# YukeWang96/GNNAdvisor_OSDI21

Hardware: AMD Instinct MI355X
Metric: aggregated edges/sec, GCN sum-aggregation SpMM (SAG) hidden=64 (higher is better)
Workload: dtype f32; 1 GPU; reddit-like power-law graph, random node order; num_nodes=232965, nnz=114623790, dim=64, partSize=128, num_parts=1008217, parallelism=single GPU, call=GNNA.SAG (pybind module, reference signature, fresh output), decider=auto/mi355x, column_phases=16, build_id=0.6.1+70ede4b55f79bb39

## Files before the change

### gnnadvisor_osdi21_amd/csrc/gnna_agg.hip

```cpp
#include <hip/hip_runtime.h>

#include <algorithm>
#include <cmath>
#include <cstdint>
#include <cstdio>

#include "gnna.h"
#include "gnna_device.h"
#include "gnna_internal.h"

namespace gnna {
namespace {


__global__ void __launch_bounds__(kBlock)
prologue_kernel(float *__restrict__ Y, size_t n_floats, int D, int ldy, const int32_t *__restrict__ p2n,
                const int32_t *__restrict__ pp, int64_t P, int32_t *flag, int32_t seq, int validate, int zero_fill,
                const int32_t *__restrict__ chk_ids, int64_t chk_n, const unsigned long long *__restrict__ chk_sum,
                int32_t *stale_flag, uint32_t *__restrict__ clear_words, int n_clear)
{
    if (blockIdx.x == 0 && (int)threadIdx.x < n_clear) clear_words[threadIdx.x] = 0u;
    const unsigned fill_blocks = chk_ids ? gridDim.x - 1 : gridDim.x;
    if (blockIdx.x >= fill_blocks) {
        if (threadIdx.x < kWave) {
// ... 261 lines not shown
    if (st.edges <= 0 || half_rows < 256.0) return 0.0;
    const double pos = std::min(23.0, 2.0 * std::log2(half_rows / 256.0));
    const int k = (int)pos;
    const double lo = st.near[k], hi = st.near[std::min(23, k + 1)];
    return (lo + (hi - lo) * (pos - k)) / st.edges;
}

int sweep_auto_phases(const gnna_tuning &t, int mode, int dim, size_t x_bytes, int64_t num_out_rows, int64_t num_in_rows,
                      const SlicePlanStats &st, int B, int num_cus, bool deterministic, int part_size)
{
    const double edges = st.edges;
    if (t.sweep != 0 || deterministic || B < 2) return 0;
    if (dim <= 32 || dim > 64 || !sweep_supports(mode, dim, x_bytes)) return 0;
    if (num_in_rows != num_out_rows || x_bytes > ((size_t)160 << 20)) return 0;
    if (edges < 300.0 * (double)std::max<int64_t>(1, num_out_rows)) return 0;
    const double cap = (double)sweep_acc_rows(dim, 1) * 0.9 * (double)std::max(8, num_cus);
    if ((double)num_out_rows > 2.0 * cap) return 0;
    if (near_share(st, (double)num_in_rows / 16.0) > 0.30) return 0;
    if (t.column_phases >= 2) return B;
    return std::max(2, std::min(std::min(16, 2 * B), std::max(2, part_size / 4)));
}

constexpr double kDenseEdgeSeconds = 9.9e-12;
constexpr double kDenseChunkSeconds = 0.97e-6;
constexpr double kDenseLaunchSeconds = 7.0e-6;
constexpr double kDenseMinSaving = 25.0e-6;
constexpr double kDenseMinShare = 0.03;

int trimmed_hubs(int H, int num_cus)
{
    const int round = kDenseTileRanks * std::max(1, num_cus);
    return (H > round && H % round != 0 && H % round < round / 4) ? H / round * round : H;
}

double dense_block_saving(double hubs, double entries, int num_cus)
{
    if (hubs <= 0.0) return 0.0;
    const double He = (double)trimmed_hubs((int)hubs, num_cus);
    const double Hp = std::ceil(He / kDenseChunkRanks) * kDenseChunkRanks;
    const double rounds = std::ceil(Hp / kDenseTileRanks / (double)std::max(1, num_cus));
    const double kept = entries * (He / hubs) * (He / hubs);
    return kept * kDenseEdgeSeconds - rounds * (Hp / kDenseChunkRanks) * kDenseChunkSeconds - kDenseLaunchSeconds;
}

bool dense_block_pays(double saving, double entries, double edges) { return saving > kDenseMinSaving && entries >= kDenseMinShare * edges; }

int sweep_phases_of_width(const gnna_tuning &t, int dim, size_t foot_bytes, size_t x_bytes, int64_t num_out_rows,
                          int64_t num_in_rows, const SlicePlanStats &st, int B, int num_cus, int partSize, int S)
{
    int Bs = sweep_auto_phases(t, MODE_SAG, dim, foot_bytes, num_out_rows, num_in_rows, st, B, num_cus, t.deterministic == 1, partSize);
    if (t.sweep == 1 && t.deterministic != 1 && sweep_supports(MODE_SAG, dim, x_bytes))
        Bs = t.column_phases >= 2 ? B : std::max(2, std::min(std::min(16, 2 * B), std::max(2, partSize / 4)));
    return std::min(Bs, S);
}

int choose_slices(const SlicePlanStats &st, size_t x_bytes, int S, uint32_t slice_rows, int64_t num_out_rows,
                  bool square, bool hinted_scattered)
{
    if (st.groups <= 0 || st.edges <= 0) return 1;
    if (!hinted_scattered) {
        if (square) {
            const double row_bytes = (double)x_bytes / ((double)slice_rows * S);
            const double half_rows = 1.75 * 1048576.0 / row_bytes;
            const bool long_rows_cached = st.edges >= 200.0 * (double)std::max<int64_t>(1, num_out_rows) && x_bytes <= (size_t)250000000;
            const bool one_line_rows = row_bytes > 64.0 && row_bytes <= 128.0;
// ... 304 lines not shown
            rc = get_packed_ids(ds, stream, db.res_plan, Bs, kWave, false, false, &res_ids, &res_off);
            if (rc != GNNA_OK) return rc;
            dense = true;
        }
        uint32_t *sync = ds->sweep_sync + (size_t)call_block_of(ds, stream, seq) * kSweepSlotWords;
        static_assert(kXcds * 16 + 2 <= kBlock, "the prologue clears the sweep counters with one block");
        rc = run_prologue(0, sync, kXcds * 16 + 2);
        if (rc != GNNA_OK) return rc;
        SweepLaunch w;
        w.mode = mode; w.X = X; w.col = column_index; w.pp = part_pointers; w.p2n = part2Node; w.Y = out;
        w.cnt = cnt; w.row_scale = row_scale; w.flag = flag; w.seq = seq; w.trust = tune.trust_canonical ? 1 : 0; w.sync = sync;
        w.P = num_parts; w.D = dim; w.ldx = ldx; w.ldy = ldy; w.S = S; w.B = Bs;
        w.relu = relu; w.num_out_rows = num_nodes;
        w.U = std::max(tune.loads_in_flight, 8);
        w.rows_with_edges = plan.stats.valid ? (int64_t)std::min((double)num_nodes, plan.stats.groups) : num_nodes;
        if (tune.groups_per_chunk > 64) w.rounds = tune.groups_per_chunk / 64;
        w.slack = tune.sweep_slack; w.wgs_per_cu = tune.blocks_per_cu;
        w.dynamic = tune.xcd_remap != 0;
        w.plain_ok = !accumulate_into_out; w.eps = eps;
        w.ids_packed = sw_ids; w.item_off = sw_off; w.packed_stale = stale_flag;
        if (dense) { w.res_col = db.res_col; w.res_pp = db.res_pp; w.res_cnt = db.res_cnt; w.res_ids_packed = res_ids; w.res_item_off = res_off; }
        t_last_phases = Bs;
        t_last_launches = 1;
        rc = launch_sweep(ds, w, stream);
        if (rc != GNNA_OK) return rc;
        if (dense) {
            rc = launch_hub_block(ds, stream, db, X, ldx, out, ldy, dim, mode == MODE_GIN, eps, row_scale, stale_flag, seq);
            if (rc != GNNA_OK) return rc;
        }
        profile_record(prof_call, 2, stream);
        return GNNA_OK;
    }

    int G = std::min(64, tune.groups_per_chunk * B);
    if (mode == MODE_EDGE && cnt && !windowed && plan.handle && plan.pinned && (plan.stats.valid || tune.sweep == 1) &&
        tune.xcd_remap != 0) {
        const int Bs = sweep_phases_of_width(tune, dim, foot_bytes, x_bytes, num_nodes, num_in_rows, plan.stats, B, ds->num_cus,
                                             partSize, S);
        if (Bs >= 2) { B = Bs; G = kWave; }
    }
    t_last_phases = B;
    StreamLaunch a;
    a.mode = mode; a.X = X; a.col = column_index; a.pp = part_pointers; a.p2n = part2Node; a.Y = out;
    a.cnt = cnt; a.row_scale = row_scale; a.flag = flag; a.seq = seq;
    if (mode == MODE_EDGE) { a.deg_row = nullptr; a.deg_col = nullptr; a.edge_w = degrees_in; }
    else { a.deg_row = degrees; a.deg_col = degrees_in; }
    a.trust = tune.trust_canonical ? 1 : 0; a.P = num_parts;
    a.D = dim; a.ldx = ldx; a.ldy = ldy; a.G = G; a.U = tune.loads_in_flight; a.S = S; a.B = B;
    a.win_lo = win_lo; a.win_hi = win_hi; a.relu = relu; a.num_out_rows = num_nodes;
    t_last_launches = 1;
// ... 206 lines not shown
    if (num_parts < 0 || num_in_rows < 0 || num_out_rows < 0 || partSize <= 0 || num_dims < 0 || (num_dims > 0 && !dims))
        return fail(GNNA_ERR_INVALID_ARGUMENT, "gnna_prepare_graph: bad argument");
    for (int i = 0; i < num_dims; i++)
        if (phases_out) phases_out[i] = 1;
    if (num_parts == 0) return GNNA_OK;
    if (!column_index || !part_pointers || !part2Node) return fail(GNNA_ERR_INVALID_ARGUMENT, "null index pointer");
    hipStream_t stream = static_cast<hipStream_t>(stream_v);
    hipStreamCaptureStatus cap = hipStreamCaptureStatusNone;
    (void)hipStreamIsCapturing(stream, &cap);
    if (cap != hipStreamCaptureStatusNone)
        return fail(GNNA_ERR_UNSUPPORTED, "gnna_prepare_graph synchronises and allocates: call it before the capture");
    DeviceState *ds = nullptr;
    int rc = get_device_state(&ds);
    if (rc != GNNA_OK) return rc;
    drain_dead_buffers();
    LaunchGuard in_flight;
    SlicePlan plan;
    rc = get_slice_plan(ds, stream, column_index, part_pointers, part2Node, num_parts, num_in_rows, true, true, &plan);
    if (rc != GNNA_OK) return rc;
    if (!plan.cnt || !plan.stats.valid) return fail(GNNA_ERR_HIP, "gnna_prepare_graph: the slice plan could not be built");
    gnna_tuning tune;
    gnna_get_tuning(&tune);
    const bool hot = plan.stats.edges >= 32.0 * (double)num_in_rows;
    size_t staged = 0, det_bytes = 0;
    std::vector<std::pair<int, int>> widths;
    for (int i = 0; i < num_dims; i++) {
        if (dims[i] <= 0) return fail(GNNA_ERR_INVALID_ARGUMENT, "gnna_prepare_graph: dims[%d] = %d", i, dims[i]);
        const int nb = column_blocks(tune, dims[i], num_in_rows, (int64_t)plan.stats.edges);
        if (nb <= 1) { widths.emplace_back(i, dims[i]); continue; }
        const int w = ((dims[i] + nb - 1) / nb + 3) / 4 * 4;
        widths.emplace_back(i, w);
        if (dims[i] % w) widths.emplace_back(i, dims[i] % w);
    }
    for (const auto &wd : widths) {
        const int i = wd.first;
        const int dim = wd.second;
        gnna_tuning t = tune;
        apply_graph_hints(column_index, dims[i], &t);
        const size_t raw = (size_t)num_in_rows * (size_t)dim * sizeof(float);
        const bool hot_rows = hot && raw <= ((size_t)1 << 30);
        const int ldx = pick_row_stride(t, dim, hot_rows, num_in_rows, true);
        const size_t x_bytes = (size_t)num_in_rows * (size_t)ldx * sizeof(float);
        const size_t foot_bytes = gather_footprint_bytes(num_in_rows, ldx, dim);
        if (hot_rows || t.gcn_prescale == 1 || ldx != dim) staged = std::max(staged, x_bytes);
        int B = 1;
        const bool can_slice = num_parts >= 1024 && num_in_rows >= 64 && foot_bytes >= ((size_t)2 << 20);
        {
            if (t.column_phases >= 2 && num_in_rows >= kMaxSlices) B = std::min(t.column_phases, kMaxSlices);
            else if (t.column_phases == 0 && can_slice && foot_bytes >= ((size_t)6 << 20))
                B = choose_slices(plan.stats, foot_bytes, plan.S, plan.slice_rows, num_out_rows, num_in_rows == num_out_rows,
                                  t.nonlocal_ids == 1);
        }
        const bool first_of_width = &wd == &widths.front() || (&wd - 1)->first != i;
        if (phases_out) phases_out[i] = first_of_width ? std::max(1, B) : std::max(phases_out[i], std::max(1, B));
        if (B >= 2 && t.pack_ids != 2 && plan.handle) {
            const int32_t *ids = nullptr; const uint32_t *off = nullptr;
            const int Bs = sweep_phases_of_width(t, dim, foot_bytes, x_bytes, num_out_rows, num_in_rows, plan.stats, B, ds->num_cus,
                                                 partSize, plan.S);
            const bool swept = Bs >= 2 && t.xcd_remap != 0;
            if (swept) rc = get_packed_ids(ds, stream, plan.handle, Bs, kWave, true, true, &ids, &off);
            if (rc == GNNA_OK && (!swept || t.gcn_prescale == 2))
                rc = get_packed_ids(ds, stream, plan.handle, B, std::max(1, std::min(kWave, t.groups_per_chunk * B)), true, true, &ids, &off);
            if (rc != GNNA_OK) return rc;
            if (phases_out && Bs >= 2) phases_out[i] = first_of_width ? Bs : std::max(phases_out[i], Bs);
            const int dense_mode = dense_block_mode();
            const bool self_swept = t.sweep == 0 && t.column_phases < 2;
            {
                DenseBlock have;
                if (plan_dense_block(plan.handle, &have) && have.off != (dense_mode == 0)) {
                    have.off = dense_mode == 0;
                    plan_set_dense_block(plan.handle, have);
                }
            }
            if (swept && ids && dense_mode != 0 && dim >= kDenseMinDim && dim <= kDenseMaxDim && num_in_rows == num_out_rows &&
                (dense_mode == 2 || self_swept)) {
                DenseBlock db;
                if (!plan_dense_block(plan.handle, &db) && db.declined_mode != dense_mode) {
                    rc = build_dense_block(ds, stream, column_index, part_pointers, part2Node, num_parts, num_in_rows,
                                           (int64_t)plan.stats.edges, dense_mode, &db);
                    if (rc != GNNA_OK) return rc;
                    if (db.buf) {
                        QuietBuilds quiet;
                        SlicePlan res;
                        rc = get_slice_plan(ds, stream, db.res_col, db.res_pp, part2Node, num_parts, num_in_rows, true, true, &res);
                        if (rc == GNNA_OK && res.cnt) { db.res_plan = res.handle; db.res_cnt = res.cnt; }
                        plan_set_dense_block(plan.handle, db);
                        if (rc != GNNA_OK) return rc;
                    } else {
                        db.declined_mode = dense_mode;
                        plan_set_dense_block(plan.handle, db);
                    }
                }
                if (db.buf && db.res_plan) {
                    QuietBuilds quiet;
                    const int32_t *rids = nullptr; const uint32_t *roff = nullptr;
                    rc = get_packed_ids(ds, stream, db.res_plan, Bs, kWave, true, true, &rids, &roff);
                    if (rc != GNNA_OK) return rc;
                }
            }
        }
        if (t.deterministic == 1 && dim >= 4) {
            const int G_eff = std::max(1, std::min(kWave, t.groups_per_chunk * std::max(1, B)));
            const size_t chunks = (size_t)((num_parts + G_eff - 1) / G_eff);
            det_bytes = std::max(det_bytes, (((chunks * 2 * (size_t)dim * sizeof(float)) + 255) & ~(size_t)255) +
                                                chunks * 2 * sizeof(int32_t));
        }
    }
    if (det_bytes) {
        void *ws = nullptr;
        rc = get_workspace(ds, stream, 2, det_bytes, &ws);
        if (rc != GNNA_OK) return rc;
    }
    if (staged) {
        void *ws = nullptr;
        rc = get_workspace(ds, stream, 1, staged, &ws);
        if (rc != GNNA_OK) return rc;
    }
    return GNNA_OK;
}

int gnna_release_graph(const int32_t *column_index)
{
    (void)release_slice_plans(column_index, false);
    return gnna_set_graph_hints(column_index, 0, 0);
}

int gnna_forget_graph(const int32_t *column_index)
{
    if (!column_index) return fail(GNNA_ERR_INVALID_ARGUMENT, "gnna_forget_graph: null (gnna_release_graph(NULL) drops everything)");
    (void)release_slice_plans(column_index, true);
    return gnna_set_graph_hints(column_index, 0, 0);
}

int gnna_forget_plans(const int32_t *column_index)
{
    if (!column_index) return fail(GNNA_ERR_INVALID_ARGUMENT, "gnna_forget_plans: null column_index");
    (void)release_slice_plans(column_index, true);
    return GNNA_OK;
}

// ... 6 lines not shown
```

### gnnadvisor_osdi21_amd/csrc/gnna_dense.hip

```cpp
#include <hip/hip_runtime.h>

#include <algorithm>
#include <cmath>
#include <cstdint>
#include <cstdio>
#include <cstdlib>
#include <vector>

#include "gnna.h"
#include "gnna_device.h"
#include "gnna_internal.h"

namespace gnna {
namespace {

constexpr int kHubBuckets = 64;
constexpr int kHubMax = 16384;
constexpr int kHubThreads = 512;
constexpr int kHubWaves = kHubThreads / kWave;
constexpr int kHubTileM = kDenseTileRanks;
constexpr int kHubKC = kDenseChunkRanks;
static_assert(kHubTileM == 32, "two MFMA tiles per workgroup");
constexpr int kHubStage = kHubKC / 32;
constexpr int kHubZeros = 64;
static_assert(kHubKC % kHubTileM == 0 && kHubKC * 16 == kHubThreads * kHubStage && (kHubTileM * 64) % kHubThreads == 0, "staging, elements per thread");
static_assert(kHubZeros >= kDenseMaxDim, "the zeros are a whole row");

__host__ __device__ inline int hub_bucket(int64_t d)
{
    if (d <= 1) return 0;
    int k = 0;
    while ((d >> (k + 1)) != 0) k++;
    const int b = 2 * k + ((d * d >= ((int64_t)1 << (2 * k + 1))) ? 1 : 0);
    return b < kHubBuckets ? b : kHubBuckets - 1;
}

__global__ void __launch_bounds__(kBlock)
hub_degree_kernel(const int32_t *__restrict__ pp, const int32_t *__restrict__ p2n, int64_t P, int64_t N, int32_t *__restrict__ deg)
{
    for (int64_t g = (int64_t)blockIdx.x * blockDim.x + threadIdx.x; g < P; g += (int64_t)gridDim.x * blockDim.x) {
        const int64_t r = p2n[g];
        const int len = pp[g + 1] - pp[g];
        if (r >= 0 && r < N && len > 0) atomicAdd(&deg[r], len);
    }
}

__global__ void __launch_bounds__(kBlock)
hub_hist_kernel(const int32_t *__restrict__ col, const int32_t *__restrict__ pp, const int32_t *__restrict__ p2n, int64_t P, int64_t N,
                const int32_t *__restrict__ deg, unsigned long long *__restrict__ hist)
// ... 95 lines not shown
__global__ void __launch_bounds__(kBlock)
hub_res_fill_kernel(const int32_t *__restrict__ col, const int32_t *__restrict__ pp, int64_t P, const uint32_t *__restrict__ taken,
                    const int32_t *__restrict__ res_pp, int32_t *__restrict__ res_col, int64_t res_nnz)
{
    const int lane = threadIdx.x & (kWave - 1);
    const int64_t wave = ((int64_t)blockIdx.x * blockDim.x + threadIdx.x) >> 6;
    const int64_t nwaves = ((int64_t)gridDim.x * blockDim.x) >> 6;
    const unsigned long long below = (1ull << lane) - 1ull;
    for (int64_t g = wave; g < P; g += nwaves) {
        const int a = pp[g], b = pp[g + 1];
        int64_t at = res_pp[g];
        for (int e0 = a; e0 < b; e0 += kWave) {
            const int e = e0 + lane;
            const bool keep = e < b && !hub_taken(taken, e);
            const unsigned long long K = __ballot(keep);
            const int64_t dst = at + __popcll(K & below);
            if (keep && dst < res_nnz) res_col[dst] = col[e];
            at += __popcll(K);
        }
    }
}

struct HubParams {
    const float *X;
    float *Y;
    const int32_t *r2n;
    const uint16_t *bm;
    const float *row_scale;
    const int32_t *stale;
    int32_t seq;
    int H_pad, D, ldx, ldy;
    int scaled;
    float eps;
};

typedef typename VecOf<4>::T HubVT;
typedef typename VecOf<4>::M HubMT;
typedef int HubIT __attribute__((ext_vector_type(4)));

constexpr int kHubFrag = 1088;
constexpr int kHubPiece = 16 * kHubFrag;
constexpr int kHubImage = 3 * kHubPiece;
static_assert(kHubKC == 128 && kHubTileM == 32 && kHubWaves == 8 && kHubStage == 4, "the shape hub_block_kernel is written for");

typedef __bf16 HubFrag __attribute__((ext_vector_type(8)));
typedef uint32_t HubU4 __attribute__((ext_vector_type(4)));
typedef uint32_t HubU2 __attribute__((ext_vector_type(2)));

__device__ __forceinline__ void hub_split(uint32_t x, uint32_t &hi, uint32_t &mid, uint32_t &lo)
{
    hi = x & 0xffff0000u;
    const float r = __uint_as_float(x) - __uint_as_float(hi);
    mid = __float_as_uint(r) & 0xffff0000u;
    lo = __float_as_uint(r - __uint_as_float(mid));
}

__device__ __forceinline__ uint32_t hub_pack(uint32_t first, uint32_t second) { return __builtin_amdgcn_perm(second, first, 0x07060302u); }

__device__ __forceinline__ HubFrag hub_ones(uint32_t bits)
{
    const uint32_t y = bits | (bits << 15);
    HubU4 v;
#pragma unroll
    for (int i = 0; i < 4; i++) v[i] = ((y >> (2 * i)) & 0x10001u) * 0x3f80u;
    return __builtin_bit_cast(HubFrag, v);
}

template <int NT, bool FULL>
__global__ void __launch_bounds__(kHubThreads)
hub_block_kernel(const HubParams p)
{
    if (*p.stale == p.seq) return;
    __shared__ __attribute__((aligned(16))) unsigned char s_x[2][kHubImage];
    static_assert(4 * kHubTileM * 64 * 4 <= kHubImage, "the partial tiles fit over the first image");
    const uint16_t *bm = p.bm;
    const int tid = (int)threadIdx.x;
    const int lane = tid & (kWave - 1);
    const int wib = __builtin_amdgcn_readfirstlane(tid >> 6);
    const int chunks = p.H_pad / kHubKC;
    const int steps = p.H_pad >> 5;
    const int D = p.D;

    const int g = 4 * (tid >> 6) + ((lane >> 3) & 1) + 2 * (lane >> 5), pc = (lane & 7) + 8 * ((lane >> 4) & 1);
    const int srow = 4 * g, spiece = 4 * pc;
    const int scol = spiece < D ? spiece : 0;
    const int wbase = ((g >> 3) * 4 + (pc >> 2)) * kHubFrag + (16 * ((g & 7) >> 1) + (pc & 3)) * 16 + 8 * (g & 1);
    const float *zero_row = reinterpret_cast<const float *>(p.r2n + p.H_pad);
    const uintptr_t zero_at = reinterpret_cast<uintptr_t>(zero_row + scol);
    auto load_piece = [&](int node) -> HubVT {
        const uintptr_t row = reinterpret_cast<uintptr_t>(p.X + (size_t)(node < 0 ? 0 : node) * (size_t)p.ldx + scol);
        const float *src = reinterpret_cast<const float *>(node < 0 ? zero_at : row);
        HubVT v;
        if constexpr (FULL) {
            v = *reinterpret_cast<const HubMT *>(src);
        } else if (spiece + 4 <= D) {
            v = *reinterpret_cast<const HubMT *>(src);
        } else {
            v = (HubVT)(0.f);
#pragma unroll
            for (int q = 0; q < 4; q++)
                if (spiece + q < D) v[q] = src[q];
        }
        return v;
    };
    struct Stage {
        HubVT r[kHubStage];
        HubIT node;
        uint32_t w;
    };
    auto fetch_ids = [&](int c, Stage &st) {
        const int cc = c < chunks ? c : chunks - 1;
        st.node = *reinterpret_cast<const HubIT *>(&p.r2n[cc * kHubKC + srow]);
    };
    auto fetch_words = [&](int c, Stage &st) {
        const int cc = c < chunks ? c : chunks - 1;
        st.w = bm[((size_t)blockIdx.x * (size_t)steps + (size_t)(cc * 4 + (wib & 3))) * 64 + (size_t)lane];
    };
    auto fetch_row = [&](int i, Stage &st) {
        st.r[i] = load_piece(st.node[i]);
    };
    auto stage_out = [&](int cc, const Stage &st, unsigned char *image) {
        uint32_t pk[3][2];
#pragma unroll
        for (int h = 0; h < 2; h++) {
            uint32_t a[3], b[3];
            hub_split(__float_as_uint(st.r[2 * h][cc]), a[0], a[1], a[2]);
            hub_split(__float_as_uint(st.r[2 * h + 1][cc]), b[0], b[1], b[2]);
#pragma unroll
            for (int i = 0; i < 3; i++) pk[i][h] = hub_pack(a[i], b[i]);
        }
#pragma unroll
        for (int i = 0; i < 3; i++) {
            HubU2 v;
            v[0] = pk[i][0];
            v[1] = pk[i][1];
            *reinterpret_cast<HubU2 *>(&image[wbase + i * kHubPiece + cc * 64]) = v;
        }
    };

    const int cs = wib & 3, ch = wib >> 2;
    const int rbase = (cs * 4 + 2 * ch) * kHubFrag + (16 * (lane >> 4) + 4 * (lane & 3) + ((lane & 15) >> 2)) * 16;
    HubVT acc_hi[2][2], acc_lo[2][2];
#pragma unroll
    for (int t = 0; t < 2; t++)
#pragma unroll
        for (int q = 0; q < 2; q++) acc_hi[t][q] = acc_lo[t][q] = (HubVT)(0.f);

    auto turn = [&](int c, Stage &L, const Stage &S) {
        const unsigned char *cur = s_x[c & 1];
        unsigned char *nxt = s_x[(c & 1) ^ 1];
        __builtin_amdgcn_sched_barrier(0);
        HubFrag b[2][3];
#pragma unroll
        for (int i = 0; i < 3; i++)
#pragma unroll
            for (int q = 0; q < 2; q++)
                if (NT == 4 || q == 0 || ch == 0) b[q][i] = *reinterpret_cast<const HubFrag *>(&cur[rbase + q * kHubFrag + i * kHubPiece]);
        HubFrag a[2];
        a[0] = hub_ones(L.w & 0xffu);
        a[1] = hub_ones((L.w >> 8) & 0xffu);
        __builtin_amdgcn_sched_barrier(0);
#pragma unroll
        for (int k = 0; k < 4; k++) {
            fetch_row(k, L);
            if (k < 3) {
#pragma unroll
                for (int q = 0; q < 2; q++)
                    if (NT == 4 || q == 0 || ch == 0) {
#pragma unroll
                        for (int t = 0; t < 2; t++) {
                            if (k == 0) acc_hi[t][q] = __builtin_amdgcn_mfma_f32_16x16x32_bf16(a[t], b[q][0], acc_hi[t][q], 0, 0, 0);
                            else acc_lo[t][q] = __builtin_amdgcn_mfma_f32_16x16x32_bf16(a[t], b[q][k], acc_lo[t][q], 0, 0, 0);
                        }
                    }
            }
            stage_out(k, S, nxt);
            __builtin_amdgcn_sched_barrier(0);
        }
        fetch_words(c + 3, L);
        fetch_ids(c + 6, L);
        __builtin_amdgcn_sched_barrier(0);
        __syncthreads();
    };
    Stage s0, s1, s2;
    fetch_ids(0, s0);
    fetch_ids(1, s1);
    fetch_ids(2, s2);
    auto fetch = [&](int c, Stage &st) {
#pragma unroll
        for (int i = 0; i < kHubStage; i++) fetch_row(i, st);
        fetch_words(c, st);
        fetch_ids(c + 3, st);
        __builtin_amdgcn_sched_barrier(0);
    };
    fetch(0, s0);
    fetch(1, s1);
    fetch(2, s2);
#pragma unroll
    for (int cc = 0; cc < 4; cc++) stage_out(cc, s0, s_x[0]);
    __builtin_amdgcn_sched_barrier(0);
    __syncthreads();
    int c = 0;
    for (; c + 3 <= chunks; c += 3) {
        turn(c, s0, s1);
        turn(c + 1, s1, s2);
        turn(c + 2, s2, s0);
    }
    if (c < chunks) {
        turn(c, s0, s1);
        if (c + 1 < chunks) turn(c + 1, s1, s2);
    }

    float *part = reinterpret_cast<float *>(&s_x[0][0]);
#pragma unroll
    for (int t = 0; t < 2; t++)
#pragma unroll
        for (int q = 0; q < 2; q++)
            if (NT == 4 || q == 0 || ch == 0) {
#pragma unroll
                for (int r = 0; r < 4; r++)
                    part[(cs * kHubTileM + t * 16 + (lane >> 4) * 4 + r) * 64 + (2 * ch + q) * 16 + (lane & 15)] =
                        __builtin_isinf(acc_hi[t][q][r]) ? acc_hi[t][q][r] : acc_hi[t][q][r] + acc_lo[t][q][r];
            }
    __syncthreads();
#pragma unroll
    for (int i = 0; i < kHubTileM * 64 / kHubThreads; i++) {
        const int idx = i * kHubThreads + tid;
        const int row = idx >> 6, col = idx & 63;
        if (col >= D) continue;
        float sum = part[idx];
#pragma unroll
        for (int s = 1; s < 4; s++) sum += part[s * kHubTileM * 64 + idx];
        const int node = p.r2n[(int)blockIdx.x * kHubTileM + row];
        if (node < 0 || sum == 0.f) continue;
        float scale = 1.f;
        if (p.scaled) {
            scale = p.eps;
            if (p.row_scale) scale *= p.row_scale[node];
        }
        float *dst = p.Y + (size_t)node * (size_t)p.ldy + col;
        *dst += sum * scale;
    }
}

int smallest_degree_of_bucket(int b)
{
    if (b <= 0) return 0;
    int64_t d = (int64_t)std::floor(std::pow(2.0, b / 2.0)) - 2;
    if (d < 1) d = 1;
    while (hub_bucket(d) < b) d++;
    return (int)std::min<int64_t>(d, 0x7fffffff);
}

struct DenseTemp {
    void *ptr = nullptr;
    ~DenseTemp() { if (ptr) { (void)hipFree(ptr); count_event(CTR_LAUNCH_FREES); } }
// ... 68 lines not shown
    e = hipMemcpyAsync(fetched.data(), hub_count, cnt_b + list_b, hipMemcpyDeviceToHost, stream);
    if (e == hipSuccess) e = hipStreamSynchronize(stream);
    if (e != hipSuccess) return fail(GNNA_ERR_HIP, "dense block (hub ids): %s", hipGetErrorString(e));
    int32_t H = fetched[0];
    if (H <= 0 || H > kHubMax) return GNNA_OK;
    const int32_t *got = fetched.data() + cnt_b / 4;
    std::vector<int32_t> ids(got, got + H), degs(got + kHubMax, got + kHubMax + H);
    if (trimmed_hubs(H, ds->num_cus) != H) {
        std::vector<int32_t> order((size_t)H);
        for (int i = 0; i < H; i++) order[(size_t)i] = i;
        std::sort(order.begin(), order.end(), [&](int32_t a, int32_t b) {
            return degs[(size_t)a] != degs[(size_t)b] ? degs[(size_t)a] > degs[(size_t)b] : ids[(size_t)a] < ids[(size_t)b];
        });
        H = trimmed_hubs(H, ds->num_cus);
        std::vector<int32_t> kept((size_t)H);
        for (int i = 0; i < H; i++) kept[(size_t)i] = ids[(size_t)order[(size_t)i]];
        ids.swap(kept);
    }
    const int H_pad = (H + kHubKC - 1) / kHubKC * kHubKC;
    std::vector<int32_t> ranks((size_t)H_pad, -1);
    std::copy(ids.begin(), ids.end(), ranks.begin());
    std::sort(ranks.begin(), ranks.begin() + H);

    const size_t r2n_b = align256((size_t)H_pad * 4 + kHubZeros * 4);
    const size_t bm_b = align256((size_t)H_pad * (size_t)H_pad / 8), rpp_b = align256((size_t)(P + 1) * 4);
    void *blk = nullptr;
    e = hipMalloc(&blk, r2n_b + bm_b + rpp_b);
    count_event(CTR_LAUNCH_MALLOCS);
    if (e != hipSuccess) { (void)hipGetLastError(); return GNNA_OK; }
    char *bb = static_cast<char *>(blk);
    int32_t *r2n = reinterpret_cast<int32_t *>(bb);
    uint32_t *bm = reinterpret_cast<uint32_t *>(bb + r2n_b);
    int32_t *res_pp = reinterpret_cast<int32_t *>(bb + r2n_b + bm_b);
    int32_t *res_col = nullptr;
    auto give_up = [&](int rc) { (void)hipStreamSynchronize(stream); (void)hipFree(blk); if (res_col) (void)hipFree(res_col); return rc; };
    e = hipMemcpy(r2n, ranks.data(), (size_t)H_pad * 4, hipMemcpyHostToDevice);
    if (e != hipSuccess) return give_up(fail(GNNA_ERR_HIP, "dense block (ranks): %s", hipGetErrorString(e)));
    (void)hipMemsetAsync(n2r, 0xff, n2r_b, stream);
    (void)hipMemsetAsync(r2n + H_pad, 0, kHubZeros * 4, stream);
    (void)hipMemsetAsync(bm, 0, bm_b, stream);
    hipLaunchKernelGGL(hub_rank_kernel, dim3((unsigned)((H + kBlock - 1) / kBlock)), dim3(kBlock), 0, stream, r2n, (int)H, N, n2r);
    hipLaunchKernelGGL(hub_bitmap_kernel, dim3(wblocks), dim3(kBlock), 0, stream, col, pp, p2n, P, N, n2r, H_pad / 32, bm, taken, taken_total);
    hipLaunchKernelGGL(hub_res_count_kernel, dim3(elementwise_grid(P + 1, ds->num_cus, 8)), dim3(kBlock), 0, stream, pp, P, taken, res_pp);
    int rc = launch_exclusive_scan(stream, res_pp, P + 1, partial);
    if (rc != GNNA_OK) return give_up(rc);
    unsigned long long entries = 0;
    e = hipMemcpyAsync(&entries, taken_total, sizeof(entries), hipMemcpyDeviceToHost, stream);
    if (e == hipSuccess) e = hipStreamSynchronize(stream);
    if (e != hipSuccess) return give_up(fail(GNNA_ERR_HIP, "dense block (bitmap): %s", hipGetErrorString(e)));
    const int64_t res_nnz = nnz - (int64_t)entries;
    if (entries == 0 || res_nnz <= 0) return give_up(GNNA_OK);
    e = hipMalloc(reinterpret_cast<void **>(&res_col), ((size_t)res_nnz + 16) * 4);
    count_event(CTR_LAUNCH_MALLOCS);
    if (e != hipSuccess) { (void)hipGetLastError(); res_col = nullptr; return give_up(GNNA_OK); }
    (void)hipMemsetAsync(res_col + res_nnz, 0, 16 * 4, stream);
    hipLaunchKernelGGL(hub_res_fill_kernel, dim3(wblocks), dim3(kBlock), 0, stream, col, pp, P, taken, res_pp, res_col, res_nnz);
    e = hipGetLastError();
    if (e == hipSuccess) e = hipStreamSynchronize(stream);
    if (e != hipSuccess) return give_up(fail(GNNA_ERR_HIP, "dense block (residual): %s", hipGetErrorString(e)));
    out->buf = blk; out->r2n = r2n; out->bm = bm; out->res_pp = res_pp; out->res_col = res_col;
    out->H = H; out->H_pad = H_pad; out->theta = theta; out->entries = (int64_t)entries; out->res_nnz = res_nnz;
    out->forced = mode == 2;
    const char *log = std::getenv("GNNA_DENSE_BLOCK_LOG");
    if (log && *log && *log != '0')
        std::fprintf(stderr, "gnna dense block: theta %d, H %d (padded %d), entries %lld of %lld edges, density %.3f\n", theta, (int)H,
                     H_pad, (long long)entries, (long long)nnz, (double)entries / ((double)H * (double)H));
    count_event(CTR_DENSE_BUILDS);
    return GNNA_OK;
}

int launch_hub_block(DeviceState *ds, hipStream_t stream, const DenseBlock &db, const float *X, int ldx, float *Y, int ldy, int dim,
                     bool scaled, float eps, const float *row_scale, const int32_t *stale_flag, int32_t seq)
{
    HubParams p;
    p.X = X; p.Y = Y; p.r2n = db.r2n; p.bm = static_cast<const uint16_t *>(db.bm); p.row_scale = row_scale;
    p.stale = stale_flag; p.seq = seq; p.H_pad = db.H_pad; p.D = dim; p.ldx = ldx; p.ldy = ldy;
    p.scaled = scaled ? 1 : 0; p.eps = eps;
    (void)ds;
    if (dim < kDenseMinDim || dim > kDenseMaxDim) return fail(GNNA_ERR_INVALID_ARGUMENT, "hub block: width %d", dim);
    const bool full = dim % 4 == 0 && ldx % 4 == 0;
    const dim3 grid((unsigned)(db.H_pad / kHubTileM)), block(kHubThreads);
    if (dim <= 48) {
        if (full) hipLaunchKernelGGL((hub_block_kernel<3, true>), grid, block, 0, stream, p);
        else hipLaunchKernelGGL((hub_block_kernel<3, false>), grid, block, 0, stream, p);
    } else {
        if (full) hipLaunchKernelGGL((hub_block_kernel<4, true>), grid, block, 0, stream, p);
        else hipLaunchKernelGGL((hub_block_kernel<4, false>), grid, block, 0, stream, p);
    }
    const int rc = launch_ok("hub block launch");
    if (rc == GNNA_OK) count_event(CTR_DENSE_LAUNCHES);
    return rc;
}

}
```

### gnnadvisor_osdi21_amd/csrc/gnna_internal.h

```cpp
#ifndef GNNA_INTERNAL_H_
#define GNNA_INTERNAL_H_

#include <hip/hip_runtime.h>

#include <atomic>
#include <cstddef>
#include <cstdint>
#include <map>
#include <utility>
#include <vector>

#include "gnna.h"
#include "gnna_launch.h"

namespace gnna {

int fail(int code, const char *fmt, ...) __attribute__((format(printf, 2, 3)));

int host_thread_budget(int cap);

void apply_graph_hints(const void *column_index, int dim, gnna_tuning *tune);

int launch_ok(const char *prefix_fmt, ...) __attribute__((format(printf, 1, 2)));
inline int xcd_remap_on()
// ... 103 lines not shown
enum { CTR_PLAN_BUILDS = 0, CTR_LAUNCH_SYNCS = 1, CTR_LAUNCH_FREES = 2, CTR_LAUNCH_MALLOCS = 3, CTR_BACKOFF_SKIPS = 4,
       CTR_SWEEP_LAUNCHES = 5, CTR_PACK_BUILDS = 6, CTR_PACKED_LAUNCHES = 7, CTR_FULL_HASHES = 8, CTR_CAPTURE_SCRATCH = 9,
       CTR_DENSE_BUILDS = 10, CTR_DENSE_LAUNCHES = 11, CTR_COUNT = 12 };
void count_event(int which);
struct QuietBuilds {
    QuietBuilds();
    ~QuietBuilds();
    QuietBuilds(const QuietBuilds &) = delete;
    QuietBuilds &operator=(const QuietBuilds &) = delete;
};

struct DenseBlock {
    void *buf = nullptr;
    const int32_t *r2n = nullptr;
    const void *bm = nullptr;
    const int32_t *res_pp = nullptr;
    int32_t *res_col = nullptr;
    const uint8_t *res_cnt = nullptr;
    void *res_plan = nullptr;
    int H = 0, H_pad = 0, theta = 0;
    int64_t entries = 0, res_nnz = 0;
    bool forced = false;
    bool off = false;
    int declined_mode = -1;
};
constexpr int kDenseTileRanks = 32, kDenseChunkRanks = 128;
constexpr int kDenseMinDim = 33, kDenseMaxDim = 64;
int trimmed_hubs(int H, int num_cus);
double dense_block_saving(double hubs, double entries, int num_cus);
bool dense_block_pays(double saving, double entries, double edges);
int dense_block_mode();
int build_dense_block(DeviceState *ds, hipStream_t stream, const int32_t *col, const int32_t *pp, const int32_t *p2n, int64_t P,
                      int64_t N, int64_t nnz, int mode, DenseBlock *out);
int launch_hub_block(DeviceState *ds, hipStream_t stream, const DenseBlock &db, const float *X, int ldx, float *Y, int ldy, int dim,
                     bool scaled, float eps, const float *row_scale, const int32_t *stale_flag, int32_t seq);
bool plan_dense_block(void *plan_handle, DenseBlock *out);
void plan_set_dense_block(void *plan_handle, const DenseBlock &db);

struct StreamLaunch {
    int mode;
    const float *X; const int32_t *col; const int32_t *pp; const int32_t *p2n; float *Y;
    const uint8_t *cnt;
    const float *row_scale;
    const float *deg_row; const float *deg_col;
    const float *A = nullptr;
    const float *edge_w = nullptr;
    const int32_t *flag; int32_t seq; int32_t trust;
    int64_t P;
    int D, ldx, G, U, S, B;
    int lda = 0;
    int ldy = 0;
    int win_lo = 0, win_hi = 0;
    bool relu = false;
    int64_t num_out_rows = 0;
    bool wide, plain_ok, xcd_remap;
    float eps;
    bool det = false;
// ... 71 lines not shown
```

Measured before the change: 89.45 billion edges/s.

## Precompute hub bf16 split image once and add taller dense hub tiles

The hub features are split into three bf16 fragments by a separate kernel that writes a pre-swizzled image to workspace before the sweep. Each hub-block workgroup then streams fragments straight from global memory instead of re-splitting X into LDS every chunk, which removes the per-workgroup conversion and the per-chunk barriers. A 64-row tile variant is picked when there are more tiles than CUs, so each B fragment feeds more MFMAs. The cost model is retuned to match, adding a fixed split-kernel cost. In exchange there is an extra launch, extra workspace, and more global traffic for the image. Whether the dense path runs at all on this graph depends on that cost model.

```diff
diff --git a/gnnadvisor_osdi21_amd/csrc/gnna_agg.hip b/gnnadvisor_osdi21_amd/csrc/gnna_agg.hip
--- a/gnnadvisor_osdi21_amd/csrc/gnna_agg.hip
+++ b/gnnadvisor_osdi21_amd/csrc/gnna_agg.hip
@@ -307,7 +307,9 @@
 }
 
 constexpr double kDenseEdgeSeconds = 9.9e-12;
-constexpr double kDenseChunkSeconds = 0.97e-6;
+constexpr double kDenseChunkSeconds = 0.73e-6;
+constexpr double kDenseTallChunkSeconds = 0.76e-6;
+constexpr double kDenseSplitSeconds = 11.0e-6;
 constexpr double kDenseLaunchSeconds = 7.0e-6;
 constexpr double kDenseMinSaving = 25.0e-6;
 constexpr double kDenseMinShare = 0.03;
@@ -323,9 +325,11 @@
     if (hubs <= 0.0) return 0.0;
     const double He = (double)trimmed_hubs((int)hubs, num_cus);
     const double Hp = std::ceil(He / kDenseChunkRanks) * kDenseChunkRanks;
-    const double rounds = std::ceil(Hp / kDenseTileRanks / (double)std::max(1, num_cus));
+    const int tile = dense_tile_ranks((int)Hp, num_cus);
+    const double rounds = std::ceil(Hp / tile / (double)std::max(1, num_cus));
+    const double t_chunk = tile == kDenseTileRanks ? kDenseChunkSeconds : kDenseTallChunkSeconds;
     const double kept = entries * (He / hubs) * (He / hubs);
-    return kept * kDenseEdgeSeconds - rounds * (Hp / kDenseChunkRanks) * kDenseChunkSeconds - kDenseLaunchSeconds;
+    return kept * kDenseEdgeSeconds - rounds * (Hp / kDenseChunkRanks) * t_chunk - kDenseSplitSeconds - kDenseLaunchSeconds;
 }
 
 bool dense_block_pays(double saving, double entries, double edges) { return saving > kDenseMinSaving && entries >= kDenseMinShare * edges; }
@@ -676,10 +680,17 @@
         if (dense) { w.res_col = db.res_col; w.res_pp = db.res_pp; w.res_cnt = db.res_cnt; w.res_ids_packed = res_ids; w.res_item_off = res_off; }
         t_last_phases = Bs;
         t_last_launches = 1;
+        void *hub_image = nullptr;
+        if (dense) {
+            rc = get_workspace(ds, stream, kSlotDenseImage, dense_image_bytes(db.H_pad), &hub_image);
+            if (rc != GNNA_OK) return rc;
+            rc = launch_hub_split(stream, db, X, ldx, dim, hub_image, stale_flag, seq);
+            if (rc != GNNA_OK) return rc;
+        }
         rc = launch_sweep(ds, w, stream);
         if (rc != GNNA_OK) return rc;
         if (dense) {
-            rc = launch_hub_block(ds, stream, db, X, ldx, out, ldy, dim, mode == MODE_GIN, eps, row_scale, stale_flag, seq);
+            rc = launch_hub_block(ds, stream, db, hub_image, out, ldy, dim, mode == MODE_GIN, eps, row_scale, stale_flag, seq);
             if (rc != GNNA_OK) return rc;
         }
         profile_record(prof_call, 2, stream);
@@ -932,7 +943,7 @@
     gnna_tuning tune;
     gnna_get_tuning(&tune);
     const bool hot = plan.stats.edges >= 32.0 * (double)num_in_rows;
-    size_t staged = 0, det_bytes = 0;
+    size_t staged = 0, det_bytes = 0, hub_image = 0;
     std::vector<std::pair<int, int>> widths;
     for (int i = 0; i < num_dims; i++) {
         if (dims[i] <= 0) return fail(GNNA_ERR_INVALID_ARGUMENT, "gnna_prepare_graph: dims[%d] = %d", i, dims[i]);
@@ -977,9 +988,13 @@
             const bool self_swept = t.sweep == 0 && t.column_phases < 2;
             {
                 DenseBlock have;
-                if (plan_dense_block(plan.handle, &have) && have.off != (dense_mode == 0)) {
-                    have.off = dense_mode == 0;
-                    plan_set_dense_block(plan.handle, have);
+                if (plan_dense_block(plan.handle, &have)) {
+                    const int tile = dense_block_tile_env(dense_mode);
+                    if (have.off != (dense_mode == 0) || have.tile != tile) {
+                        have.off = dense_mode == 0;
+                        have.tile = tile;
+                        plan_set_dense_block(plan.handle, have);
+                    }
                 }
             }
             if (swept && ids && dense_mode != 0 && dim >= kDenseMinDim && dim <= kDenseMaxDim && num_in_rows == num_out_rows &&
@@ -1006,6 +1021,7 @@
                     const int32_t *rids = nullptr; const uint32_t *roff = nullptr;
                     rc = get_packed_ids(ds, stream, db.res_plan, Bs, kWave, true, true, &rids, &roff);
                     if (rc != GNNA_OK) return rc;
+                    hub_image = std::max(hub_image, dense_image_bytes(db.H_pad));
                 }
             }
         }
@@ -1026,6 +1042,11 @@
         rc = get_workspace(ds, stream, 1, staged, &ws);
         if (rc != GNNA_OK) return rc;
     }
+    if (hub_image) {
+        void *ws = nullptr;
+        rc = get_workspace(ds, stream, kSlotDenseImage, hub_image, &ws);
+        if (rc != GNNA_OK) return rc;
+    }
     return GNNA_OK;
 }
 
diff --git a/gnnadvisor_osdi21_amd/csrc/gnna_dense.hip b/gnnadvisor_osdi21_amd/csrc/gnna_dense.hip
--- a/gnnadvisor_osdi21_amd/csrc/gnna_dense.hip
+++ b/gnnadvisor_osdi21_amd/csrc/gnna_dense.hip
@@ -20,11 +20,10 @@
 constexpr int kHubWaves = kHubThreads / kWave;
 constexpr int kHubTileM = kDenseTileRanks;
 constexpr int kHubKC = kDenseChunkRanks;
-static_assert(kHubTileM == 32, "two MFMA tiles per workgroup");
-constexpr int kHubStage = kHubKC / 32;
-constexpr int kHubZeros = 64;
-static_assert(kHubKC % kHubTileM == 0 && kHubKC * 16 == kHubThreads * kHubStage && (kHubTileM * 64) % kHubThreads == 0, "staging, elements per thread");
-static_assert(kHubZeros >= kDenseMaxDim, "the zeros are a whole row");
+static_assert(kHubTileM == 32, "a tile row of the bitmap per 32 destination ranks");
+constexpr int kSplitThreads = 128;
+static_assert(kHubKC % (2 * kHubTileM) == 0 && (kHubTileM * 64) % kHubThreads == 0, "whole tiles per chunk, elements per thread");
+static_assert(kDenseMaxDim <= 64, "the split image holds 64 columns");
 
 __host__ __device__ inline int hub_bucket(int64_t d)
 {
@@ -166,26 +165,34 @@
 }
 
 struct HubParams {
-    const float *X;
     float *Y;
     const int32_t *r2n;
     const uint16_t *bm;
+    const unsigned char *img;
     const float *row_scale;
     const int32_t *stale;
     int32_t seq;
-    int H_pad, D, ldx, ldy;
+    int H_pad, D, ldy;
     int scaled;
     float eps;
 };
 
+struct SplitParams {
+    const float *X;
+    const int32_t *r2n;
+    unsigned char *img;
+    const int32_t *stale;
+    int32_t seq;
+    int D, ldx;
+};
+
 typedef typename VecOf<4>::T HubVT;
-typedef typename VecOf<4>::M HubMT;
 typedef int HubIT __attribute__((ext_vector_type(4)));
 
-constexpr int kHubFrag = 1088;
+constexpr int kHubFrag = 1024;
 constexpr int kHubPiece = 16 * kHubFrag;
 constexpr int kHubImage = 3 * kHubPiece;
-static_assert(kHubKC == 128 && kHubTileM == 32 && kHubWaves == 8 && kHubStage == 4, "the shape hub_block_kernel is written for");
+static_assert(kHubKC == 128 && kHubTileM == 32 && kHubWaves == 8, "the shape hub_block_kernel is written for");
 
 typedef __bf16 HubFrag __attribute__((ext_vector_type(8)));
 typedef uint32_t HubU4 __attribute__((ext_vector_type(4)));
@@ -210,172 +217,166 @@
     return __builtin_bit_cast(HubFrag, v);
 }
 
-template <int NT, bool FULL>
+template <bool FULL>
+__global__ void __launch_bounds__(kSplitThreads)
+hub_split_kernel(const SplitParams p)
+{
+    if (*p.stale == p.seq) return;
+    __shared__ __attribute__((aligned(16))) unsigned char s_img[3 * 4 * kHubFrag];
+    const int t = (int)threadIdx.x;
+    const int g = t >> 4, pc = t & 15;
+    const int step = (int)blockIdx.x;
+    const int D = p.D;
+    const HubIT node = *reinterpret_cast<const HubIT *>(&p.r2n[step * 32 + 4 * g]);
+    HubVT v[4];
+#pragma unroll
+    for (int k = 0; k < 4; k++) {
+        const int nd = node[k];
+        const float *src = p.X + (size_t)(nd < 0 ? 0 : nd) * (size_t)p.ldx + 4 * pc;
+        HubVT x = (HubVT)(0.f);
+        if (nd >= 0) {
+            if constexpr (FULL) {
+                if (4 * pc < D) x = *reinterpret_cast<const HubVT *>(src);
+            } else {
+#pragma unroll
+                for (int q = 0; q < 4; q++)
+                    if (4 * pc + q < D) x[q] = src[q];
+            }
+        }
+        v[k] = x;
+    }
+    const int wbase = (pc >> 2) * kHubFrag + (16 * (g >> 1) + 4 * (pc & 3)) * 16 + 8 * (g & 1);
+#pragma unroll
+    for (int cc = 0; cc < 4; cc++) {
+        uint32_t pk[3][2];
+#pragma unroll
+        for (int h = 0; h < 2; h++) {
+            uint32_t a[3], b[3];
+            hub_split(__float_as_uint(v[2 * h][cc]), a[0], a[1], a[2]);
+            hub_split(__float_as_uint(v[2 * h + 1][cc]), b[0], b[1], b[2]);
+#pragma unroll
+            for (int i = 0; i < 3; i++) pk[i][h] = hub_pack(a[i], b[i]);
+        }
+#pragma unroll
+        for (int i = 0; i < 3; i++) {
+            HubU2 o;
+            o[0] = pk[i][0];
+            o[1] = pk[i][1];
+            *reinterpret_cast<HubU2 *>(&s_img[wbase + i * 4 * kHubFrag + cc * 16]) = o;
+        }
+    }
+    __syncthreads();
+    unsigned char *out = p.img + (size_t)(step >> 2) * kHubImage + (size_t)(step & 3) * 4 * kHubFrag;
+#pragma unroll
+    for (int u = 0; u < 3 * 4 * kHubFrag / 16 / kSplitThreads; u++) {
+        const int idx = u * kSplitThreads + t;
+        const int i = idx >> 8, off = (idx & 255) * 16;
+        *reinterpret_cast<HubU4 *>(&out[i * kHubPiece + off]) = *reinterpret_cast<const HubU4 *>(&s_img[i * 4 * kHubFrag + off]);
+    }
+}
+
+template <int NT, int TM>
 __global__ void __launch_bounds__(kHubThreads)
 hub_block_kernel(const HubParams p)
 {
     if (*p.stale == p.seq) return;
-    __shared__ __attribute__((aligned(16))) unsigned char s_x[2][kHubImage];
-    static_assert(4 * kHubTileM * 64 * 4 <= kHubImage, "the partial tiles fit over the first image");
-    const uint16_t *bm = p.bm;
+    constexpr int TR = TM / 32;
+    static_assert((TM == kHubTileM || TM == 2 * kHubTileM) && (NT == 3 || NT == 4), "tile shapes");
+    __shared__ __attribute__((aligned(16))) float s_part[4 * TM * 64];
     const int tid = (int)threadIdx.x;
     const int lane = tid & (kWave - 1);
     const int wib = __builtin_amdgcn_readfirstlane(tid >> 6);
     const int chunks = p.H_pad / kHubKC;
     const int steps = p.H_pad >> 5;
     const int D = p.D;
-
-    const int g = 4 * (tid >> 6) + ((lane >> 3) & 1) + 2 * (lane >> 5), pc = (lane & 7) + 8 * ((lane >> 4) & 1);
-    const int srow = 4 * g, spiece = 4 * pc;
-    const int scol = spiece < D ? spiece : 0;
-    const int wbase = ((g >> 3) * 4 + (pc >> 2)) * kHubFrag + (16 * ((g & 7) >> 1) + (pc & 3)) * 16 + 8 * (g & 1);
-    const float *zero_row = reinterpret_cast<const float *>(p.r2n + p.H_pad);
-    const uintptr_t zero_at = reinterpret_cast<uintptr_t>(zero_row + scol);
-    auto load_piece = [&](int node) -> HubVT {
-        const uintptr_t row = reinterpret_cast<uintptr_t>(p.X + (size_t)(node < 0 ? 0 : node) * (size_t)p.ldx + scol);
-        const float *src = reinterpret_cast<const float *>(node < 0 ? zero_at : row);
-        HubVT v;
-        if constexpr (FULL) {
-            v = *reinterpret_cast<const HubMT *>(src);
-        } else if (spiece + 4 <= D) {
-            v = *reinterpret_cast<const HubMT *>(src);
-        } else {
-            v = (HubVT)(0.f);
-#pragma unroll
-            for (int q = 0; q < 4; q++)
-                if (spiece + q < D) v[q] = src[q];
-        }
-        return v;
+    const int cs = wib & 3, ch = wib >> 2;
+    const bool two = NT == 4 || ch == 0;
+    const unsigned char *frag0 = p.img + (size_t)(cs * 4 + 2 * ch) * kHubFrag + (size_t)lane * 16;
+    const uint16_t *word0 = p.bm + ((size_t)blockIdx.x * TR * (size_t)steps + (size_t)cs) * 64 + (size_t)lane;
+    struct Stage {
+        HubFrag b[2][3];
+        uint32_t w[TR];
     };
-    struct Stage {
-        HubVT r[kHubStage];
-        HubIT node;
-        uint32_t w;
-    };
-    auto fetch_ids = [&](int c, Stage &st) {
-        const int cc = c < chunks ? c : chunks - 1;
-        st.node = *reinterpret_cast<const HubIT *>(&p.r2n[cc * kHubKC + srow]);
+    auto fetch_piece = [&](int c, int i, Stage &st) {
+        const unsigned char *src = frag0 + (size_t)(c < chunks ? c : chunks - 1) * kHubImage + i * kHubPiece;
+        st.b[0][i] = *reinterpret_cast<const HubFrag *>(src);
+        if (two) st.b[1][i] = *reinterpret_cast<const HubFrag *>(src + kHubFrag);
     };
     auto fetch_words = [&](int c, Stage &st) {
         const int cc = c < chunks ? c : chunks - 1;
-        st.w = bm[((size_t)blockIdx.x * (size_t)steps + (size_t)(cc * 4 + (wib & 3))) * 64 + (size_t)lane];
+#pragma unroll
+        for (int tr = 0; tr < TR; tr++) st.w[tr] = word0[((size_t)tr * (size_t)steps + (size_t)(cc * 4)) * 64];
     };
-    auto fetch_row = [&](int i, Stage &st) {
-        st.r[i] = load_piece(st.node[i]);
-    };
-    auto stage_out = [&](int cc, const Stage &st, unsigned char *image) {
-        uint32_t pk[3][2];
-#pragma unroll
-        for (int h = 0; h < 2; h++) {
-            uint32_t a[3], b[3];
-            hub_split(__float_as_uint(st.r[2 * h][cc]), a[0], a[1], a[2]);
-            hub_split(__float_as_uint(st.r[2 * h + 1][cc]), b[0], b[1], b[2]);
-#pragma unroll
-            for (int i = 0; i < 3; i++) pk[i][h] = hub_pack(a[i], b[i]);
-        }
-#pragma unroll
-        for (int i = 0; i < 3; i++) {
-            HubU2 v;
-            v[0] = pk[i][0];
-            v[1] = pk[i][1];
-            *reinterpret_cast<HubU2 *>(&image[wbase + i * kHubPiece + cc * 64]) = v;
-        }
-    };
-
-    const int cs = wib & 3, ch = wib >> 2;
-    const int rbase = (cs * 4 + 2 * ch) * kHubFrag + (16 * (lane >> 4) + 4 * (lane & 3) + ((lane & 15) >> 2)) * 16;
-    HubVT acc_hi[2][2], acc_lo[2][2];
-#pragma unroll
-    for (int t = 0; t < 2; t++)
+    HubVT acc_hi[2 * TR][2], acc_lo[2 * TR][2];
+#pragma unroll
+    for (int t = 0; t < 2 * TR; t++)
 #pragma unroll
         for (int q = 0; q < 2; q++) acc_hi[t][q] = acc_lo[t][q] = (HubVT)(0.f);
 
-    auto turn = [&](int c, Stage &L, const Stage &S) {
-        const unsigned char *cur = s_x[c & 1];
-        unsigned char *nxt = s_x[(c & 1) ^ 1];
+    auto turn = [&](int c, Stage &st) {
+        HubFrag a[2 * TR];
+#pragma unroll
+        for (int t = 0; t < 2 * TR; t++) a[t] = hub_ones((st.w[t >> 1] >> (8 * (t & 1))) & 0xffu);
         __builtin_amdgcn_sched_barrier(0);
-        HubFrag b[2][3];
-#pragma unroll
-        for (int i = 0; i < 3; i++)
+#pragma unroll
+        for (int k = 0; k < 3; k++) {
 #pragma unroll
             for (int q = 0; q < 2; q++)
-                if (NT == 4 || q == 0 || ch == 0) b[q][i] = *reinterpret_cast<const HubFrag *>(&cur[rbase + q * kHubFrag + i * kHubPiece]);
-        HubFrag a[2];
-        a[0] = hub_ones(L.w & 0xffu);
-        a[1] = hub_ones((L.w >> 8) & 0xffu);
+                if (q == 0 || two) {
+#pragma unroll
+                    for (int t = 0; t < 2 * TR; t++) {
+                        if (k == 0) acc_hi[t][q] = __builtin_amdgcn_mfma_f32_16x16x32_bf16(a[t], st.b[q][0], acc_hi[t][q], 0, 0, 0);
+                        else acc_lo[t][q] = __builtin_amdgcn_mfma_f32_16x16x32_bf16(a[t], st.b[q][k], acc_lo[t][q], 0, 0, 0);
+                    }
+                }
+            fetch_piece(c + 3, k, st);
+            __builtin_amdgcn_sched_barrier(0);
+        }
+        fetch_words(c + 3, st);
         __builtin_amdgcn_sched_barrier(0);
-#pragma unroll
-        for (int k = 0; k < 4; k++) {
-            fetch_row(k, L);
-            if (k < 3) {
-#pragma unroll
-                for (int q = 0; q < 2; q++)
-                    if (NT == 4 || q == 0 || ch == 0) {
-#pragma unroll
-                        for (int t = 0; t < 2; t++) {
-                            if (k == 0) acc_hi[t][q] = __builtin_amdgcn_mfma_f32_16x16x32_bf16(a[t], b[q][0], acc_hi[t][q], 0, 0, 0);
-                            else acc_lo[t][q] = __builtin_amdgcn_mfma_f32_16x16x32_bf16(a[t], b[q][k], acc_lo[t][q], 0, 0, 0);
-                        }
-                    }
-            }
-            stage_out(k, S, nxt);
-            __builtin_amdgcn_sched_barrier(0);
-        }
-        fetch_words(c + 3, L);
-        fetch_ids(c + 6, L);
-        __builtin_amdgcn_sched_barrier(0);
-        __syncthreads();
     };
     Stage s0, s1, s2;
-    fetch_ids(0, s0);
-    fetch_ids(1, s1);
-    fetch_ids(2, s2);
     auto fetch = [&](int c, Stage &st) {
 #pragma unroll
-        for (int i = 0; i < kHubStage; i++) fetch_row(i, st);
+        for (int i = 0; i < 3; i++) fetch_piece(c, i, st);
         fetch_words(c, st);
-        fetch_ids(c + 3, st);
         __builtin_amdgcn_sched_barrier(0);
     };
     fetch(0, s0);
     fetch(1, s1);
     fetch(2, s2);
-#pragma unroll
-    for (int cc = 0; cc < 4; cc++) stage_out(cc, s0, s_x[0]);
-    __builtin_amdgcn_sched_barrier(0);
-    __syncthreads();
     int c = 0;
     for (; c + 3 <= chunks; c += 3) {
-        turn(c, s0, s1);
-        turn(c + 1, s1, s2);
-        turn(c + 2, s2, s0);
+        turn(c, s0);
+        turn(c + 1, s1);
+        turn(c + 2, s2);
     }
     if (c < chunks) {
-        turn(c, s0, s1);
-        if (c + 1 < chunks) turn(c + 1, s1, s2);
-    }
-
-    float *part = reinterpret_cast<float *>(&s_x[0][0]);
-#pragma unroll
-    for (int t = 0; t < 2; t++)
+        turn(c, s0);
+        if (c + 1 < chunks) turn(c + 1, s1);
+    }
+
+    float *part = s_part;
+#pragma unroll
+    for (int t = 0; t < 2 * TR; t++)
 #pragma unroll
         for (int q = 0; q < 2; q++)
-            if (NT == 4 || q == 0 || ch == 0) {
+            if (q == 0 || two) {
 #pragma unroll
                 for (int r = 0; r < 4; r++)
-                    part[(cs * kHubTileM + t * 16 + (lane >> 4) * 4 + r) * 64 + (2 * ch + q) * 16 + (lane & 15)] =
+                    part[(cs * TM + t * 16 + (lane >> 4) * 4 + r) * 64 + (2 * ch + q) * 16 + (lane & 15)] =
                         __builtin_isinf(acc_hi[t][q][r]) ? acc_hi[t][q][r] : acc_hi[t][q][r] + acc_lo[t][q][r];
             }
     __syncthreads();
 #pragma unroll
-    for (int i = 0; i < kHubTileM * 64 / kHubThreads; i++) {
+    for (int i = 0; i < TM * 64 / kHubThreads; i++) {
         const int idx = i * kHubThreads + tid;
         const int row = idx >> 6, col = idx & 63;
         if (col >= D) continue;
         float sum = part[idx];
 #pragma unroll
-        for (int s = 1; s < 4; s++) sum += part[s * kHubTileM * 64 + idx];
-        const int node = p.r2n[(int)blockIdx.x * kHubTileM + row];
+        for (int s = 1; s < 4; s++) sum += part[s * TM * 64 + idx];
+        const int node = p.r2n[(int)blockIdx.x * TM + row];
         if (node < 0 || sum == 0.f) continue;
         float scale = 1.f;
         if (p.scaled) {
@@ -490,7 +491,7 @@
     std::copy(ids.begin(), ids.end(), ranks.begin());
     std::sort(ranks.begin(), ranks.begin() + H);
 
-    const size_t r2n_b = align256((size_t)H_pad * 4 + kHubZeros * 4);
+    const size_t r2n_b = align256((size_t)H_pad * 4);
     const size_t bm_b = align256((size_t)H_pad * (size_t)H_pad / 8), rpp_b = align256((size_t)(P + 1) * 4);
     void *blk = nullptr;
     e = hipMalloc(&blk, r2n_b + bm_b + rpp_b);
@@ -505,7 +506,6 @@
     e = hipMemcpy(r2n, ranks.data(), (size_t)H_pad * 4, hipMemcpyHostToDevice);
     if (e != hipSuccess) return give_up(fail(GNNA_ERR_HIP, "dense block (ranks): %s", hipGetErrorString(e)));
     (void)hipMemsetAsync(n2r, 0xff, n2r_b, stream);
-    (void)hipMemsetAsync(r2n + H_pad, 0, kHubZeros * 4, stream);
     (void)hipMemsetAsync(bm, 0, bm_b, stream);
     hipLaunchKernelGGL(hub_rank_kernel, dim3((unsigned)((H + kBlock - 1) / kBlock)), dim3(kBlock), 0, stream, r2n, (int)H, N, n2r);
     hipLaunchKernelGGL(hub_bitmap_kernel, dim3(wblocks), dim3(kBlock), 0, stream, col, pp, p2n, P, N, n2r, H_pad / 32, bm, taken, taken_total);
@@ -529,6 +529,7 @@
     out->buf = blk; out->r2n = r2n; out->bm = bm; out->res_pp = res_pp; out->res_col = res_col;
     out->H = H; out->H_pad = H_pad; out->theta = theta; out->entries = (int64_t)entries; out->res_nnz = res_nnz;
     out->forced = mode == 2;
+    out->tile = dense_block_tile_env(mode);
     const char *log = std::getenv("GNNA_DENSE_BLOCK_LOG");
     if (log && *log && *log != '0')
         std::fprintf(stderr, "gnna dense block: theta %d, H %d (padded %d), entries %lld of %lld edges, density %.3f\n", theta, (int)H,
@@ -537,23 +538,42 @@
     return GNNA_OK;
 }
 
-int launch_hub_block(DeviceState *ds, hipStream_t stream, const DenseBlock &db, const float *X, int ldx, float *Y, int ldy, int dim,
+int dense_block_tile_env(int mode)
+{
+    const char *s = mode == 2 ? std::getenv("GNNA_DENSE_BLOCK_TILE") : nullptr;
+    const int v = s && *s ? std::atoi(s) : 0;
+    return v == kHubTileM || v == 2 * kHubTileM ? v : 0;
+}
+
+int launch_hub_split(hipStream_t stream, const DenseBlock &db, const float *X, int ldx, int dim, void *image, const int32_t *stale_flag,
+                     int32_t seq)
+{
+    if (dim < kDenseMinDim || dim > kDenseMaxDim) return fail(GNNA_ERR_INVALID_ARGUMENT, "hub block: width %d", dim);
+    SplitParams p;
+    p.X = X; p.r2n = db.r2n; p.img = static_cast<unsigned char *>(image); p.stale = stale_flag; p.seq = seq; p.D = dim; p.ldx = ldx;
+    const bool full = dim % 4 == 0 && ldx % 4 == 0 && (reinterpret_cast<uintptr_t>(X) & 15) == 0;
+    const dim3 grid((unsigned)(db.H_pad / 32)), block(kSplitThreads);
+    if (full) hipLaunchKernelGGL((hub_split_kernel<true>), grid, block, 0, stream, p);
+    else hipLaunchKernelGGL((hub_split_kernel<false>), grid, block, 0, stream, p);
+    return launch_ok("hub split launch");
+}
+
+int launch_hub_block(DeviceState *ds, hipStream_t stream, const DenseBlock &db, const void *image, float *Y, int ldy, int dim,
                      bool scaled, float eps, const float *row_scale, const int32_t *stale_flag, int32_t seq)
 {
     HubParams p;
-    p.X = X; p.Y = Y; p.r2n = db.r2n; p.bm = static_cast<const uint16_t *>(db.bm); p.row_scale = row_scale;
-    p.stale = stale_flag; p.seq = seq; p.H_pad = db.H_pad; p.D = dim; p.ldx = ldx; p.ldy = ldy;
+    p.Y = Y; p.r2n = db.r2n; p.bm = static_cast<const uint16_t *>(db.bm); p.img = static_cast<const unsigned char *>(image);
+    p.row_scale = row_scale; p.stale = stale_flag; p.seq = seq; p.H_pad = db.H_pad; p.D = dim; p.ldy = ldy;
     p.scaled = scaled ? 1 : 0; p.eps = eps;
-    (void)ds;
     if (dim < kDenseMinDim || dim > kDenseMaxDim) return fail(GNNA_ERR_INVALID_ARGUMENT, "hub block: width %d", dim);
-    const bool full = dim % 4 == 0 && ldx % 4 == 0;
-    const dim3 grid((unsigned)(db.H_pad / kHubTileM)), block(kHubThreads);
-    if (dim <= 48) {
-        if (full) hipLaunchKernelGGL((hub_block_kernel<3, true>), grid, block, 0, stream, p);
-        else hipLaunchKernelGGL((hub_block_kernel<3, false>), grid, block, 0, stream, p);
+    const int tile = dense_tile_ranks(db.H_pad, ds->num_cus, db.tile);
+    const dim3 grid((unsigned)(db.H_pad / tile)), block(kHubThreads);
+    if (tile == kHubTileM) {
+        if (dim <= 48) hipLaunchKernelGGL((hub_block_kernel<3, kHubTileM>), grid, block, 0, stream, p);
+        else hipLaunchKernelGGL((hub_block_kernel<4, kHubTileM>), grid, block, 0, stream, p);
     } else {
-        if (full) hipLaunchKernelGGL((hub_block_kernel<4, true>), grid, block, 0, stream, p);
-        else hipLaunchKernelGGL((hub_block_kernel<4, false>), grid, block, 0, stream, p);
+        if (dim <= 48) hipLaunchKernelGGL((hub_block_kernel<3, 2 * kHubTileM>), grid, block, 0, stream, p);
+        else hipLaunchKernelGGL((hub_block_kernel<4, 2 * kHubTileM>), grid, block, 0, stream, p);
     }
     const int rc = launch_ok("hub block launch");
     if (rc == GNNA_OK) count_event(CTR_DENSE_LAUNCHES);
diff --git a/gnnadvisor_osdi21_amd/csrc/gnna_internal.h b/gnnadvisor_osdi21_amd/csrc/gnna_internal.h
--- a/gnnadvisor_osdi21_amd/csrc/gnna_internal.h
+++ b/gnnadvisor_osdi21_amd/csrc/gnna_internal.h
@@ -149,9 +149,17 @@
     int64_t entries = 0, res_nnz = 0;
     bool forced = false;
     bool off = false;
+    int tile = 0;
     int declined_mode = -1;
 };
 constexpr int kDenseTileRanks = 32, kDenseChunkRanks = 128;
+inline int dense_tile_ranks(int H_pad, int num_cus, int forced = 0)
+{
+    if (forced == kDenseTileRanks || forced == 2 * kDenseTileRanks) return forced;
+    return H_pad / kDenseTileRanks <= (num_cus > 1 ? num_cus : 1) ? kDenseTileRanks : 2 * kDenseTileRanks;
+}
+constexpr int kSlotDenseImage = 18;
+inline size_t dense_image_bytes(int H_pad) { return (size_t)H_pad * 3 * 64 * 2; }
 constexpr int kDenseMinDim = 33, kDenseMaxDim = 64;
 int trimmed_hubs(int H, int num_cus);
 double dense_block_saving(double hubs, double entries, int num_cus);
@@ -159,7 +167,10 @@
 int dense_block_mode();
 int build_dense_block(DeviceState *ds, hipStream_t stream, const int32_t *col, const int32_t *pp, const int32_t *p2n, int64_t P,
                       int64_t N, int64_t nnz, int mode, DenseBlock *out);
-int launch_hub_block(DeviceState *ds, hipStream_t stream, const DenseBlock &db, const float *X, int ldx, float *Y, int ldy, int dim,
+int dense_block_tile_env(int mode);
+int launch_hub_split(hipStream_t stream, const DenseBlock &db, const float *X, int ldx, int dim, void *image, const int32_t *stale_flag,
+                     int32_t seq);
+int launch_hub_block(DeviceState *ds, hipStream_t stream, const DenseBlock &db, const void *image, float *Y, int ldy, int dim,
                      bool scaled, float eps, const float *row_scale, const int32_t *stale_flag, int32_t seq);
 bool plan_dense_block(void *plan_handle, DenseBlock *out);
 void plan_set_dense_block(void *plan_handle, const DenseBlock &db);
```

Result: faster. 92.20 billion edges/s, median of 6 (+3.1%).
